# szpajder/dumphfdl

Hardware: AMD Instinct MI355X
Metric: wideband I/Q Msamples/s (cf32 ingest -> decoded HFDL PDUs) at fixed channel count (higher is better)
Workload: dtype f32

## Files before the change

### dumphfdl_amd/csrc/demod_core.h

```cpp
#pragma once
#include <hip/hip_runtime.h>
#include "demod_logic.h"
#include "demod_lds.h"

namespace hfdl {

constexpr int DM_WAVES = 4, DM_THREADS = 64 * DM_WAVES;

__device__ __forceinline__ float dpp_row_shr1(float old, float src)
{
	return __int_as_float(__builtin_amdgcn_update_dpp(__float_as_int(old), __float_as_int(src), 0x111, 0xf, 0xf, false));
}
__device__ __forceinline__ float dpp_row_shl1(float old, float src)
{
	return __int_as_float(__builtin_amdgcn_update_dpp(__float_as_int(old), __float_as_int(src), 0x101, 0xf, 0xf, false));
}
__device__ __forceinline__ float dpp_row_shl2(float old, float src)
{
	return __int_as_float(__builtin_amdgcn_update_dpp(__float_as_int(old), __float_as_int(src), 0x102, 0xf, 0xf, false));
}
__device__ __forceinline__ float dpp_row_ror1(float src)
{
	return __int_as_float(__builtin_amdgcn_update_dpp(0, __float_as_int(src), 0x121, 0xf, 0xf, false));
}
// ... 116 lines not shown
		for (int j = 0; j < D_RS_TAPS; j++) {
			const cf x = ring[(i - j) & DM_IN_MASK];
			ar += h[j] * x.x;
			ai += h[j] * x.y;
		}
		cf v; v.x = ar; v.y = ai;
		io.rs[k & DM_MASK] = v;
		if (TAPS) io.tap_resampled[k] = v;
	}
}


struct SymsyncRegs {
	float rate, del, tau, bf, q, qhat, v1;
	int b, decim, j;
	int valid_from;
};

__device__ __forceinline__ void symsync_load(SymsyncRegs &r, const ChanScalars &s, const ChanArrays &a, const BlockIo &io, int lane)
{
	if (lane < SS_HIST) {
		cf v; v.x = 0.f; v.y = 0.f;
		if (lane < D_SS_TAPS) v = a.ss_dmf[lane == 0 ? 0 : D_SS_TAPS - lane];
		io.mf[-1 - lane] = v;
	}
	r.rate = s.ss_rate; r.del = s.ss_del; r.tau = s.ss_tau; r.bf = s.ss_bf; r.q = s.ss_q; r.qhat = s.ss_qhat; r.v1 = s.ss_v1;
	r.b = s.ss_b; r.decim = (int)s.ss_decim; r.j = 0;
	r.valid_from = s.ss_head;
}

__device__ __forceinline__ void symsync_restart(SymsyncRegs &r, const DemodShared &sh, int k0)
{
	r.rate = 1.5f; r.del = 1.5f; r.tau = 0.f; r.bf = 0.f; r.q = 0.f; r.qhat = 0.f; r.v1 = 0.f;
	r.b = 0; r.decim = 0;
	r.j = k0 > 0 ? (int)sh.cum[(k0 - 1) & DM_MASK] : 0;
	r.valid_from = k0;
}

__device__ __forceinline__ void symsync_store(const SymsyncRegs &r, ChanScalars &s, ChanArrays &a, const BlockIo &io, int n_out, int lane)
{
	if (lane < D_SS_TAPS) a.ss_dmf[lane == 0 ? 0 : D_SS_TAPS - lane] = io.mf[((n_out - 1) & DM_MASK) - lane];
	if (lane == 0) {
		s.ss_rate = r.rate; s.ss_del = r.del; s.ss_tau = r.tau; s.ss_bf = r.bf; s.ss_q = r.q; s.ss_qhat = r.qhat; s.ss_v1 = r.v1;
		s.ss_b = r.b; s.ss_decim = (uint32_t)r.decim;
		const int vf = r.valid_from - n_out;
		s.ss_head = vf < -64 ? -64 : vf;
	}
}

template <bool MASKED>
__device__ __forceinline__ void symsync_chunk(SymsyncRegs &r, const DemodConst &T, const BlockIo &io, const DemodShared &sh, int k0, int k1, int lane)
{
	const int row = lane >> 4, t = lane & 15;
	const float *base = (const float *)(io.mf - (k0 & ~DM_MASK) - t) + (row & 1);
	int bi = r.b < 0 ? 0 : (r.b >= D_SS_NPFB ? D_SS_NPFB - 1 : r.b);
	float2 h = sh.sstab[bi * 64 + lane];
	float w_lo = base[2 * k0], w_hi = base[2 * (k0 - 16)];
	const bool out_lane = lane == 15 || lane == 31;
	float *const out_base = out_lane ? (float *)sh.outq + (lane == 31 ? 1 : 0) : sh.sink + lane;
	const int out_stride = out_lane ? 2 : 0;
	int cum_v = 0;
	for (int k = k0; k < k1; k++) {
		const float n_lo = base[2 * (k + 1)], n_hi = base[2 * (k + 1 - 16)];
		if (r.b < D_SS_NPFB) {
			float wl = w_lo, wh = w_hi;
			if (MASKED && k - (D_SS_TAPS - 1) < r.valid_from && row < 2) {
				if (k - t < r.valid_from) wl = 0.f;
				if (k - t - 16 < r.valid_from) wh = 0.f;
			}
			int produced = 0;
			do {
				const float p = row_scan_sum(h.x * wl + h.y * wh);
				if (__builtin_expect(r.j < sh.outq_cap, 1)) out_base[out_stride * (r.j & (OUTQ_RING - 1))] = div3(p);
				r.j++;
				if (r.decim == 2) {
					r.decim = 0;
					const float mx = lane_value(p, 15), my = lane_value(p, 31);
					const float dx = lane_value(p, 47), dy = lane_value(p, 63);
					float q = mx * dx + my * dy;
					q = q > 1.0f ? 1.0f : (q < -1.0f ? -1.0f : q);
					r.q = q;
					const float v0 = q - T.lf_a1 * r.v1;
					r.qhat = T.lf_b0 * v0;
					r.v1 = v0;
					r.rate += T.ss_rate_adj * r.qhat;
					r.del = r.rate + r.qhat;
				}
				r.decim++;
				r.tau += r.del;
				r.bf = r.tau * (float)D_SS_NPFB;
				r.b = (int)roundf(r.bf);
				produced++;
				if (r.b < D_SS_NPFB) h = sh.sstab[(r.b < 0 ? 0 : r.b) * 64 + lane];
			} while (r.b < D_SS_NPFB && produced < 4);
		}
		r.tau -= 1.0f;
		r.bf -= (float)D_SS_NPFB;
		r.b -= D_SS_NPFB;
		bi = r.b < 0 ? 0 : (r.b >= D_SS_NPFB ? D_SS_NPFB - 1 : r.b);
		h = sh.sstab[bi * 64 + lane];
		cum_v = (lane == k - k0) ? (r.j < 65535 ? r.j : 65535) : cum_v;
		w_lo = n_lo; w_hi = n_hi;
	}
	if (lane < k1 - k0) sh.cum[(k0 + lane) & DM_MASK] = (uint16_t)cum_v;
}


struct CarrierRegs {
	float eu, ev, ex2, ewx, ewy;
	float px, py;
#ifdef HFDL_DM_PROBE
	unsigned long long pa = 0, pb = 0, pc = 0;
#endif
};

struct LaneSlicer {
	float px, py;
	int lane;
	__device__ __forceinline__ uint32_t operator()(int arity, cf x, float *phase_error) const
	{
		uint32_t sym;
		cf xh;
		if (arity == 1) {
			sym = (x.x > 0) ? 0 : 1;
			xh.x = sym ? -1.0f : 1.0f; xh.y = 0.0f;
		} else {
			const int M = 1 << arity, base = M - 2;
			const bool mine = lane >= base && lane < base + M;
			const float d = mine ? x.x * px + x.y * py : -1.0f;
			const float best = lane_value(row_scan_max(d), 15);
			const unsigned long long hit = __builtin_amdgcn_fcmpf(d, best, 1 );
			int win = hit ? (int)__builtin_ctzll(hit) : base;
			const uint32_t lin = (uint32_t)(win - base);
			sym = lin ^ (lin >> 1);
			xh.x = lane_value(px, win); xh.y = lane_value(py, win);
		}
		if (phase_error) *phase_error = x.y * xh.x - x.x * xh.y;
		return sym;
	}
};

__device__ __forceinline__ void carrier_load(CarrierRegs &c, const ChanScalars &s, const ChanArrays &a, const DemodConst &T, int lane)
{
	c.px = lane < 16 ? T.psk_pts[2 * lane] : 0.f;
	c.py = lane < 16 ? T.psk_pts[2 * lane + 1] : 0.f;
	const int t = (lane & 15) - 1;
	const bool act = t >= 0 && lane < 32, row1 = (lane >> 4) & 1;
	int j = s.eq_head + t; if (j >= D_EQ) j -= D_EQ;
	const cf e = act ? a.eq_buf[j] : cf{0.f, 0.f};
	c.eu = row1 ? e.y : e.x;
	c.ev = row1 ? -e.x : e.y;
	c.ex2 = act ? a.eq_x2[j] : 0.f;
	const cf w = act ? a.eq_w[t] : cf{0.f, 0.f};
	c.ewx = w.x; c.ewy = w.y;
}
// ... 299 lines not shown
	if (reset_at >= 0) {
		s.ev_flags = 0;
		s.sample_cnt = cnt0 + (uint64_t)reset_at + 1u;
		return k0 + reset_at;
	}
	if (kdone < n) catch_up(n - 1);
	s.sample_cnt = cnt0 + (uint64_t)n;
	return -1;
}


template <bool TAPS>
__device__ inline int demod_block(ChanArrays &a, const DemodConst &T, const BlockIo &io, const DemodShared &sh, const DemodInput &in)
{
	const int tid = (int)threadIdx.x, wave = tid >> 6, lane = tid & 63;
	ChanScalars &S = *sh.S;
	unsigned long long tR0 = __builtin_amdgcn_s_memtime();

	const uint32_t rs_phase = S.rs_phase;
	const int n_in = in.n_in;
	const uint64_t total = (uint64_t)n_in << 24;
	int n_out = 0;
	if ((uint64_t)rs_phase < total) n_out = (int)((total - rs_phase + T.rs_step - 1) / T.rs_step);
	if (n_out > io.cap - 4) n_out = io.cap - 4;
	auto need = [&](int k_end) {
		return k_end >= n_out ? n_in : (int)(((uint64_t)rs_phase + (uint64_t)(k_end - 1) * T.rs_step) >> 24) + 1;
	};
	auto resampler_store = [&]() {
		cf nh;
		if (lane < D_RS_TAPS - 1) nh = in.ring[(n_in - 1 - lane) & DM_IN_MASK];
		__builtin_amdgcn_wave_barrier();
		if (lane < D_RS_TAPS - 1) a.rs_hist[lane] = nh;
		if (lane == 0) {
			S.rs_phase = (uint32_t)((uint64_t)rs_phase + (uint64_t)n_out * T.rs_step - total);
			if (TAPS) io.tap_counts[0] = n_out;
		}
	};

	if (tid < D_RS_TAPS - 1) in.ring[(-1 - tid) & DM_IN_MASK] = a.rs_hist[tid];
	if (wave == 1 && lane < D_MF - 1) io.agc[(-1 - lane) & DM_AGC_MASK] = a.mf_hist[lane];
	const int rs0 = n_out < DM_CHUNK ? n_out : DM_CHUNK;
	int in_loaded = need(rs0 + 2 * DM_CHUNK);
	for (int g = tid; g < in_loaded; g += DM_THREADS) in.ring[g & DM_IN_MASK] = input_sample(in, g);
	if (TAPS && tid == 0) io.tap_counts[1] = 0;
	__syncthreads();
	if (wave == 3) resample_outputs<TAPS>(rs_phase, T, io, in.ring, 0, rs0, lane);
	__syncthreads();
	if (n_out < 1) {
		if (wave == 3) resampler_store();
		return 0;
	}

	unsigned long long tP0 = __builtin_amdgcn_s_memtime();
	unsigned long long busy = 0;
	int nsym = 0;
#ifdef HFDL_DM_PROBE
	unsigned long long cr_probe[3] = { 0, 0, 0 };
#endif
	PipeProgress pp;
	pp.rs_ready = rs0;
	if (wave == 3) {
		for (int step = 0; pp.s3_done < n_out; step++) {
			int *mb = sh.mbox + 8 * (step & 1);
			int to = pp.rs_ready;
			if (to < n_out) {
				to = to + DM_CHUNK < n_out ? to + DM_CHUNK : n_out;
				if (to > pp.s3_done + DM_RS_AHEAD) to = pp.s3_done + DM_RS_AHEAD;
				const int hi = need(to + 2 * DM_CHUNK < n_out ? to + 2 * DM_CHUNK : n_out);
				cf nx[2];
#pragma unroll
				for (int u = 0; u < 2; u++) {
					const int g = in_loaded + 64 * u + lane;
					nx[u] = g < hi ? input_sample(in, g) : cf{0.f, 0.f};
				}
				resample_outputs<TAPS>(rs_phase, T, io, in.ring, pp.rs_ready, to, lane);
#pragma unroll
				for (int u = 0; u < 2; u++) {
					const int g = in_loaded + 64 * u + lane;
					if (g < hi) in.ring[g & DM_IN_MASK] = nx[u];
				}
				for (int g = in_loaded + 128 + lane; g < hi; g += 64) in.ring[g & DM_IN_MASK] = input_sample(in, g);
				if (hi > in_loaded) in_loaded = hi;
			}
			if (lane == 0) mb[4] = to;
			__syncthreads();
			pp.read(mb);
		}
		resampler_store();
	} else if (wave == 0) {
		float agc_g = S.agc_g, agc_y2 = S.agc_y2;
		for (int step = 0; pp.s3_done < n_out; step++) {
			int *mb = sh.mbox + 8 * (step & 1);
			int to = pp.mf_ready + DM_CHUNK < pp.rs_ready ? pp.mf_ready + DM_CHUNK : pp.rs_ready;
			if (to > pp.s3_done + DM_MF_AHEAD) to = pp.s3_done + DM_MF_AHEAD;
			if (to > pp.mf_ready) agc_mf_chunk<TAPS>(agc_g, agc_y2, T, io, pp.mf_ready, to, lane); else to = pp.mf_ready;
			if (lane == 0) mb[0] = to;
			__syncthreads();
			pp.read(mb);
		}
		cf nh;
		if (lane < D_MF - 1) nh = io.agc[(n_out - 1 - lane) & DM_AGC_MASK];
		__builtin_amdgcn_wave_barrier();
		if (lane < D_MF - 1) a.mf_hist[lane] = nh;
		if (lane == 0) { S.agc_g = agc_g; S.agc_y2 = agc_y2; }
	} else if (wave == 1) {
		SymsyncRegs ss;
		symsync_load(ss, S, a, io, lane);
		__builtin_amdgcn_fence(__ATOMIC_RELEASE, "wavefront");
		__builtin_amdgcn_wave_barrier();
		for (int step = 0; pp.s3_done < n_out; step++) {
			int *mb = sh.mbox + 8 * (step & 1);
			const unsigned long long tb = TAPS ? __builtin_amdgcn_s_memtime() : 0ull;
			if (pp.restart) symsync_restart(ss, sh, pp.ss_ready);
			int to = pp.ss_ready + DM_CHUNK < pp.mf_ready ? pp.ss_ready + DM_CHUNK : pp.mf_ready;
			if (to > pp.s3_done + 2 * DM_CHUNK) to = pp.s3_done + 2 * DM_CHUNK;
			if (to < pp.ss_ready) to = pp.ss_ready;
			for (int k0 = pp.ss_ready; k0 < to;) {
				const int k1 = (k0 | DM_MASK) + 1 < to ? (k0 | DM_MASK) + 1 : to;
				if (__builtin_expect(k0 - (D_SS_TAPS - 1) < ss.valid_from, 0)) symsync_chunk<true>(ss, T, io, sh, k0, k1, lane);
				else symsync_chunk<false>(ss, T, io, sh, k0, k1, lane);
				k0 = k1;
			}
			if (lane == 0) mb[1] = to;
			if (TAPS) busy += __builtin_amdgcn_s_memtime() - tb;
			__syncthreads();
			pp.read(mb);
		}
		if (pp.restart) symsync_restart(ss, sh, n_out);
		symsync_store(ss, S, a, io, n_out, lane);
	} else {
		CarrierRegs cr;
		ChanScalars s3 = S;
		s3.ev_flags = 0;
		carrier_load(cr, s3, a, T, lane);
		for (int step = 0; pp.s3_done < n_out; step++) {
			int *mb = sh.mbox + 8 * (step & 1);
			const unsigned long long tb = TAPS ? __builtin_amdgcn_s_memtime() : 0ull;
			int to = pp.s3_done + DM_CHUNK < pp.ss_ready ? pp.s3_done + DM_CHUNK : pp.ss_ready;
			int reset_at = -1;
			if (to > pp.s3_done) reset_at = carrier_chunk<TAPS>(cr, s3, a, T, io, sh, pp.s3_done, to, nsym, lane); else to = pp.s3_done;
			if (lane == 0) { mb[2] = reset_at >= 0 ? reset_at + 1 : to; mb[3] = reset_at >= 0; }
			if (TAPS) busy += __builtin_amdgcn_s_memtime() - tb;
			__syncthreads();
			pp.read(mb);
		}
		carrier_store(cr, a, lane);
#ifdef HFDL_DM_PROBE
		cr_probe[0] = cr.pa; cr_probe[1] = cr.pb; cr_probe[2] = cr.pc;
#endif
		if (lane == 0) {
			S.phi = s3.phi; S.dphi = s3.dphi; S.err = s3.err;
			S.eq_x2sum = s3.eq_x2sum; S.eq_count = s3.eq_count; S.eq_full = s3.eq_full; S.eq_head = 0;
			S.bits_hi = s3.bits_hi; S.bits_lo = s3.bits_lo;
			S.training_n = s3.training_n; S.data_n = s3.data_n; S.use_data = s3.use_data; S.data_slot = s3.data_slot;
			S.symbol_cnt = s3.symbol_cnt; S.sample_cnt = s3.sample_cnt;
			S.s_state = s3.s_state; S.fr_state = s3.fr_state; S.cur_arity = s3.cur_arity;
			S.symbols_wanted = s3.symbols_wanted; S.T_idx = s3.T_idx;
			S.bitmask = s3.bitmask; S.symsync_out_idx = s3.symsync_out_idx; S.nf_clk = s3.nf_clk;
			S.frame_symbol_cnt = s3.frame_symbol_cnt; S.signal_level = s3.signal_level;
			S.noise_floor = s3.noise_floor;
			S.ev_flags = 0;
			if (TAPS) io.tap_counts[1] = nsym;
		}
	}
	unsigned long long tP1 = __builtin_amdgcn_s_memtime();
	if (TAPS) {
		if (tid == 0) { io.tap_level[io.cap - 4] = (float)(tP0 - tR0); io.tap_level[io.cap - 3] = (float)(tP1 - tP0); }
		if (wave == 1 && lane == 0) io.tap_level[io.cap - 2] = (float)busy;
		if (wave == 2 && lane == 0) io.tap_level[io.cap - 1] = (float)busy;
#ifdef HFDL_DM_PROBE
		__syncthreads();
		if (wave == 2 && lane == 0) { io.tap_level[io.cap - 4] = (float)cr_probe[0]; io.tap_level[io.cap - 3] = (float)cr_probe[1]; io.tap_level[io.cap - 2] = (float)cr_probe[2]; }
#endif
	}
	return n_out;
}

}
```

### dumphfdl_amd/csrc/frontend_query.cpp

```cpp
#include <cstdarg>
#include <cstdio>
#include <cstring>
#include <mutex>
#include "frontend.h"

using namespace hfdl;

static thread_local char g_err[512] = "";

int hfdl::fail(int code, const char *fmt, ...)
{
	va_list ap;
	va_start(ap, fmt);
	vsnprintf(g_err, sizeof(g_err), fmt, ap);
	va_end(ap);
	return code;
}

int hfdl::fail_hip(hipError_t e, bool alloc, const char *expr, const char *file, int line)
{
	return fail(alloc && e == hipErrorOutOfMemory ? HFDL_GPU_ENOMEM : HFDL_GPU_EHIP, "%s: %s (%s:%d)", expr, hipGetErrorString(e), file, line);
}

extern "C" const char *hfdl_gpu_last_error(void) { return g_err; }
// ... 196 lines not shown
	if (!fe || !out) return fail(HFDL_GPU_EINVAL, "null argument");
	memset(out, 0, sizeof(*out));
	out->blocks = fe->blocks;
	out->pdus_taken = fe->demod.taken;
	out->pdus_dropped = fe->demod.dropped;
	out->pdu_ring_capacity = (uint32_t)fe->demod.pdu_cap;
	return 0;
}

extern "C" int hfdl_gpu_frontend_enable_taps(hfdl_gpu_frontend *fe, int enable)
{
	if (int rc = sync_to_read(fe)) return rc;
	fe->demod.taps_enabled = enable != 0;
	return 0;
}

extern "C" int hfdl_gpu_frontend_read_tap_block(hfdl_gpu_frontend *fe, int what, int32_t channel, int32_t back, float *dst, size_t cap, size_t *n_floats)
{
	if (int rc = sync_to_read(fe, dst && n_floats)) return rc;
	const Geometry &g = fe->geo;
	if (back < 0 || back > fe->last_index) return fail(HFDL_GPU_ERANGE, "block %d back is not held any more (%d are)", back, fe->last_index);
	if (back && what != HFDL_GPU_TAP_SPECTRUM && what != HFDL_GPU_TAP_CHAN_OUT && what != HFDL_GPU_TAP_NCO_PHASORS)
		return fail(HFDL_GPU_EINVAL, "tap %d holds the last launch only", what);
	const int slot = fe->last_slot - back, index = fe->last_index - back;
	if ((what != HFDL_GPU_TAP_SPECTRUM || fe->nrx > 1) && (channel < 0 || channel >= g.nch)) return fail(HFDL_GPU_EINVAL, "channel out of range");
	const void *src = nullptr;
	size_t nf = 0;
	switch (what) {
	case HFDL_GPU_TAP_SPECTRUM:
		src = fe->spec_slot(fe->last_set, index) + (fe->nrx > 1 ? (size_t)fe->rx_of[(size_t)channel] * (size_t)g.n : 0);
		nf = 2 * (size_t)g.n;
		break;
	case HFDL_GPU_TAP_FILTER: {
		if (2 * (size_t)g.n > cap) return fail(HFDL_GPU_ERANGE, "tap needs %zu floats, buffer holds %zu", 2 * (size_t)g.n, cap);
		DevBuf plain;
		HIP_TRY(plain.alloc(sizeof(float2) * (size_t)g.n));
		launch_tap_extract(fe->d_taps, g, fe->slot_of(channel), plain.as<float2>(), fe->stream);
		HIP_TRY(hipStreamSynchronize(fe->stream));
		HIP_TRY(hipMemcpy(dst, plain.p, sizeof(float2) * (size_t)g.n, hipMemcpyDeviceToHost));
		*n_floats = 2 * (size_t)g.n;
		return 0; }
	case HFDL_GPU_TAP_CHAN_OUT: {
		int cnt = 0;
		HIP_TRY(hipMemcpy(&cnt, fe->cnt_slot(slot) + channel, sizeof(cnt), hipMemcpyDeviceToHost));
		src = fe->chan_slot(slot) + (size_t)channel * g.outs; nf = 2 * (size_t)cnt; break; }
	case HFDL_GPU_TAP_NCO_PHASORS: {
		int cnt = 0;
		HIP_TRY(hipMemcpy(&cnt, fe->cnt_slot(slot) + channel, sizeof(cnt), hipMemcpyDeviceToHost));
		if (2 * (size_t)cnt > cap) return fail(HFDL_GPU_ERANGE, "tap needs %zu floats, buffer holds %zu", 2 * (size_t)cnt, cap);
		if (cnt) HIP_TRY(hipMemcpy2D(dst, sizeof(float2), fe->ph_slot(fe->last_set, index) + channel, sizeof(float2) * (size_t)g.nch, sizeof(float2), (size_t)cnt, hipMemcpyDeviceToHost));
		*n_floats = 2 * (size_t)cnt;
		return 0; }
	case HFDL_GPU_TAP_PHASE_CYCLES: src = fe->demod.d_tap_lvl + (size_t)channel * fe->demod.cap + fe->demod.cap - 4; nf = 4; break;
	default:
		if (int rc = fe->demod.tap(what, channel, &src, &nf)) return rc;
	}
	if (nf > cap) return fail(HFDL_GPU_ERANGE, "tap needs %zu floats, buffer holds %zu", nf, cap);
	if (nf) HIP_TRY(hipMemcpy(dst, src, sizeof(float) * nf, hipMemcpyDeviceToHost));
	*n_floats = nf;
	return 0;
}

extern "C" int hfdl_gpu_frontend_read_tap(hfdl_gpu_frontend *fe, int what, int32_t channel, float *dst, size_t cap, size_t *n_floats)
{
	return hfdl_gpu_frontend_read_tap_block(fe, what, channel, 0, dst, cap, n_floats);
}


static_assert(HFDL_GPU_SPECTRUM_HANN == SPECMON_HANN && HFDL_GPU_SPECTRUM_MAXHOLD == SPECMON_MAXHOLD, "include/hfdl_gpu.h and spectrum.h name the same flags");
static_assert(HFDL_GPU_RECEIVERS_MAX <= 64, "SpecmonJob::fresh is one bit per receiver");

extern "C" int hfdl_gpu_frontend_spectrum_enable(hfdl_gpu_frontend *fe, int32_t bins, uint32_t flags)
{
	if (!fe) return fail(HFDL_GPU_EINVAL, "null argument");
	if (flags & ~(HFDL_GPU_SPECTRUM_HANN | HFDL_GPU_SPECTRUM_MAXHOLD)) return fail(HFDL_GPU_EINVAL, "unknown spectrum flags 0x%x", flags);
	if (bins != 0 && (bins < 16 || (bins & (bins - 1)) != 0)) return fail(HFDL_GPU_EINVAL, "spectrum bins %d: a power of two >= 16 (or 0 = off)", bins);
	if (bins > fe->geo.n / 16) return fail(HFDL_GPU_ERANGE, "spectrum bins %d: at most fft_size / 16 = %d", bins, fe->geo.n / 16);
	HIP_TRY(hipSetDevice(fe->device));
	if (fe->mon) (void)hipEventSynchronize(fe->mon->ev);
	fe->mon.reset();
	if (bins == 0) return 0;
	const size_t nb = (size_t)bins, K = (size_t)fe->nrx;
	auto mon = std::make_unique<SpectrumMonitor>();
	hipError_t e = mon->acc.alloc(sizeof(float2) * nb * K);
	if (e == hipSuccess && (flags & HFDL_GPU_SPECTRUM_MAXHOLD)) e = mon->peak.alloc(sizeof(float) * nb * K);
	if (e == hipSuccess) e = mon->host.alloc(3 * nb);
	if (e == hipSuccess) e = mon->ev.create(EV_NO_TIMING);
	if (e != hipSuccess) return fail(e == hipErrorOutOfMemory ? HFDL_GPU_ENOMEM : HFDL_GPU_EHIP, "spectrum monitor buffers: %s", hipGetErrorString(e));
	mon->bins = bins;
	mon->flags = flags;
	mon->fresh = ~(uint64_t)0;
	mon->blocks.assign(K, 0);
	mon->first.assign(K, 0);
	fe->mon = std::move(mon);
	return 0;
}

extern "C" int hfdl_gpu_frontend_spectrum_read(hfdl_gpu_frontend *fe, int32_t rx, float *mean, float *peak, int32_t cap,
		uint64_t *blocks, uint64_t *first_block, int reset)
{
	if (!fe || !mean || !blocks || !first_block) return fail(HFDL_GPU_EINVAL, "null argument");
	SpectrumMonitor *mon = fe->mon.get();
	if (!mon) return fail(HFDL_GPU_EINVAL, "the spectrum monitor is off: hfdl_gpu_frontend_spectrum_enable() first");
	if (rx < 0 || rx >= fe->nrx) return fail(HFDL_GPU_EINVAL, "receiver %d out of range (%d receivers)", rx, fe->nrx);
	if (peak && !(mon->flags & HFDL_GPU_SPECTRUM_MAXHOLD)) return fail(HFDL_GPU_EINVAL, "peak asked for, but the monitor was enabled without HFDL_GPU_SPECTRUM_MAXHOLD");
	if (cap < mon->bins) return fail(HFDL_GPU_ERANGE, "%d bands, buffer holds %d", mon->bins, cap);
// ... 20 lines not shown
```

### dumphfdl_amd/frontend.py

```python
import ctypes as C
import os
import sys
import numpy as np

_HERE = os.path.dirname(os.path.abspath(__file__))
PDU_MAX_OCTETS = 960

TAP_SPECTRUM, TAP_FILTER, TAP_CHAN_OUT, TAP_RESAMPLED, TAP_MF_OUT, TAP_SYMBOLS, TAP_AGC_LEVEL, TAP_PHASE_CYCLES, TAP_NCO_PHASORS = range(1, 10)


SFMT_CF32, SFMT_CS16, SFMT_CU8 = 0, 1, 2
FCS_GOOD, FCS_BAD, FCS_TOO_SHORT = 0, 1, 2
KIND_SPDU, KIND_MPDU_DOWNLINK, KIND_MPDU_UPLINK = 0, 1, 2


class GpuError(RuntimeError):
    pass


class Geometry(C.Structure):
    _fields_ = [(n, C.c_int32) for n in (
        "sample_rate", "decimation", "pre_decimation", "post_decimation", "taps_length", "overlap_length",
        "fft_size", "fft_inv_size", "input_size", "post_input_size", "scrap", "outputs_per_block",
        "channels", "fold_slices")] + [("transition_bw", C.c_float), ("resamp_rate", C.c_float), ("max_outputs_per_block", C.c_int32), ("demod_batch", C.c_int32), ("fold_batch", C.c_int32),
                                       ("prefetch_depth", C.c_int32), ("fold_rows", C.c_int32)]


class Pdu(C.Structure):
    _fields_ = [("channel", C.c_int32), ("freq", C.c_int32), ("mode", C.c_int32), ("bit_rate", C.c_int32),
                ("len", C.c_int32), ("freq_err_hz", C.c_float), ("rssi_db", C.c_float), ("noise_floor_db", C.c_float),
                ("slot", C.c_char), ("fcs_status", C.c_uint8), ("pdu_kind", C.c_uint8), ("hdr_len", C.c_uint16),
                ("sample_index", C.c_uint64),
                ("train_bits_bad", C.c_int32), ("train_bits_total", C.c_int32),
                ("lpdus_processed", C.c_uint8), ("lpdus_good", C.c_uint8), ("lpdus_bad_fcs", C.c_uint8), ("lpdus_too_short", C.c_uint8),
                ("lpdus_truncated", C.c_uint8), ("lpdu_pad", C.c_uint8 * 3),
                ("octets", C.c_uint8 * PDU_MAX_OCTETS)]


class ChannelStats(C.Structure):
    _fields_ = [("freq", C.c_int32), ("a2_found", C.c_uint32), ("m1_found", C.c_uint32), ("m1_not_found", C.c_uint32),
                ("frames", C.c_uint32), ("noise_floor_db", C.c_float), ("agc_level", C.c_float), ("costas_dphi", C.c_float),
                ("framer_state", C.c_int32), ("sample_cnt", C.c_uint64), ("symbol_cnt", C.c_uint64),
                ("a1_found", C.c_uint32), ("a1_corr_avg", C.c_float), ("a2_corr_avg", C.c_float), ("m1_corr_avg", C.c_float),
                ("train_bits_bad", C.c_uint32), ("train_bits_total", C.c_uint32)]


class FrontendCounters(C.Structure):
    _fields_ = [("blocks", C.c_uint64), ("pdus_taken", C.c_uint32), ("pdus_dropped", C.c_uint32), ("pdu_ring_capacity", C.c_uint32)]


def lib_path():
    return os.environ.get("HFDL_GPU_LIB") or os.path.join(_HERE, "libhfdl_gpu.so")


def lab_lib_path():
    return os.environ.get("HFDL_GPU_LAB_LIB") or os.path.join(_HERE, "libhfdl_gpu_lab.so")


_lib = None
_lab = None

# ... 214 lines not shown
            _check(rc, self._L)
        return bool(rc)

    def input_done_upto(self, host_block):
        _check(self._L.hfdl_gpu_frontend_input_done_upto(self._h, C.c_uint64(host_block)), self._L)

    def sync(self):
        _check(self._L.hfdl_gpu_frontend_sync(self._h), self._L)

    def poll_pdus_raw(self, max_pdus=4096, max_in_flight=0):
        buf = (Pdu * max_pdus)()
        n = C.c_int32(0)
        if max_in_flight:
            _check(self._L.hfdl_gpu_frontend_poll_pdus_ready(self._h, buf, max_pdus, C.byref(n), max_in_flight), self._L)
        else:
            _check(self._L.hfdl_gpu_frontend_poll_pdus(self._h, buf, max_pdus, C.byref(n)), self._L)
        return buf, n.value

    @staticmethod
    def pdus_to_dicts(buf, n):
        out = []
        for i in range(n):
            p = buf[i]
            out.append(dict(channel=p.channel, freq=p.freq, mode=p.mode, bit_rate=p.bit_rate,
                            octets=bytes(p.octets[:p.len]), freq_err_hz=p.freq_err_hz, rssi_db=p.rssi_db,
                            noise_floor_db=p.noise_floor_db, slot=p.slot.decode(), sample_index=p.sample_index,
                            fcs_status=p.fcs_status, pdu_kind=p.pdu_kind, hdr_len=p.hdr_len,
                            train_bits_bad=p.train_bits_bad, train_bits_total=p.train_bits_total,
                            lpdus=(p.lpdus_processed, p.lpdus_good, p.lpdus_bad_fcs, p.lpdus_too_short, p.lpdus_truncated)))
        return out

    def poll_pdus(self, max_pdus=4096, max_in_flight=0):
        return self.pdus_to_dicts(*self.poll_pdus_raw(max_pdus, max_in_flight))

    def counters(self):
        c = FrontendCounters()
        _check(self._L.hfdl_gpu_frontend_counters(self._h, C.byref(c)), self._L)
        return {n: getattr(c, n) for n, _ in FrontendCounters._fields_}

    def all_channel_stats(self):
        nch = self.geometry.channels
        buf = (ChannelStats * nch)()
        n = C.c_int32(0)
        _check(self._L.hfdl_gpu_frontend_all_channel_stats(self._h, buf, nch, C.byref(n)), self._L)
        return [{k: getattr(buf[i], k) for k, _ in ChannelStats._fields_} for i in range(n.value)]

    def read_tap(self, what, channel=0, back=0):
        g = self.geometry
        cap = 2 * g.fft_size if what in (TAP_SPECTRUM, TAP_FILTER) else 2 * (g.post_input_size + 64) * max(1, g.demod_batch)
        buf = np.empty(cap, np.float32)
        n = C.c_size_t(0)
        _check(self._L.hfdl_gpu_frontend_read_tap_block(self._h, what, channel, back, _p(buf), cap, C.byref(n)), self._L)
        out = buf[:n.value].copy()
        return out if what in (TAP_AGC_LEVEL, TAP_PHASE_CYCLES) else out.view(np.complex64)

    def enable_taps(self, enable=True):
        _check(self._L.hfdl_gpu_frontend_enable_taps(self._h, int(enable)), self._L)

    def channel_stats(self, channel):
        st = ChannelStats()
        _check(self._L.hfdl_gpu_frontend_channel_stats(self._h, channel, C.byref(st)), self._L)
        return {n: getattr(st, n) for n, _ in ChannelStats._fields_}

    def reset_timers(self, enable=True):
        _check(self._L.hfdl_gpu_frontend_reset_timers(self._h, int(enable)), self._L)

    def fold_time_ms(self):
        ms = C.c_double(0)
        n = C.c_int64(0)
        _check(self._L.hfdl_gpu_frontend_fold_time_ms(self._h, C.byref(ms), C.byref(n)), self._L)
        return ms.value, n.value

    def fold_blocks(self):
        n = C.c_int64(0)
        _check(self._L.hfdl_gpu_frontend_fold_blocks(self._h, C.byref(n)), self._L)
        return n.value

    def fold_launch_shapes(self):
        c = (C.c_int64 * (FOLD_BATCH_MAX + 1))()
        _check(self._L.hfdl_gpu_frontend_fold_launch_shapes(self._h, C.byref(c), None), self._L)
        return {nb: int(c[nb]) for nb in range(1, FOLD_BATCH_MAX + 1) if c[nb]}

    def fold_launch_times(self):
        c, ms = (C.c_int64 * (FOLD_BATCH_MAX + 1))(), (C.c_double * (FOLD_BATCH_MAX + 1))()
        _check(self._L.hfdl_gpu_frontend_fold_launch_shapes(self._h, C.byref(c), C.byref(ms)), self._L)
        return {nb: (int(c[nb]), float(ms[nb])) for nb in range(1, FOLD_BATCH_MAX + 1) if c[nb]}

    def stage_times(self):
        ms, n = (C.c_double * 5)(), (C.c_int64 * 5)()
        _check(self._L.hfdl_gpu_frontend_stage_times(self._h, C.byref(ms), C.byref(n)), self._L)
        return {k: (ms[i], int(n[i])) for i, k in enumerate(("fft", "fold", "ifft", "demod", "decode"))}

    def fold_variant_probe(self, variant, nb, reps=3):
        avg, best, chk = C.c_double(0), C.c_double(0), C.c_uint64(0)
        _check(self._L.hfdl_gpu_lab_fold_variant_probe(self._h, variant, nb, reps, C.byref(avg), C.byref(best), C.byref(chk)), self._L)
        return avg.value, best.value, chk.value

    def demod_time_ms(self):
        ms = C.c_double(0)
        n = C.c_int64(0)
        nb = C.c_int64(0)
        _check(self._L.hfdl_gpu_frontend_demod_time_ms(self._h, C.byref(ms), C.byref(n), C.byref(nb)), self._L)
        return ms.value, n.value, nb.value

    def step_period_ms(self):
        v = C.c_double(0)
        _check(self._L.hfdl_gpu_frontend_step_period_ms(self._h, C.byref(v)), self._L)
# ... 185 lines not shown
```

### include/hfdl_gpu.h

```cpp
#ifndef HFDL_GPU_H
#define HFDL_GPU_H
#include <stdint.h>
#include <stddef.h>

#ifdef __cplusplus
extern "C" {
#endif

#define HFDL_GPU_EINVAL   (-1)
#define HFDL_GPU_ENODEV   (-2)
#define HFDL_GPU_ENOMEM   (-3)
#define HFDL_GPU_EHIP     (-4)
#define HFDL_GPU_ERANGE   (-5)

#define HFDL_GPU_PDU_MAX_OCTETS 960

#define HFDL_GPU_FCS_GOOD      0
#define HFDL_GPU_FCS_BAD       1
#define HFDL_GPU_FCS_TOO_SHORT 2
#define HFDL_GPU_KIND_SPDU          0
#define HFDL_GPU_KIND_MPDU_DOWNLINK 1
#define HFDL_GPU_KIND_MPDU_UPLINK   2

typedef struct hfdl_gpu_frontend hfdl_gpu_frontend;
// ... 56 lines not shown
int  hfdl_gpu_frontend_push_block(hfdl_gpu_frontend *fe, const float *iq, size_t nsamples, int on_device);
int  hfdl_gpu_frontend_input_done(hfdl_gpu_frontend *fe);
int  hfdl_gpu_frontend_input_done_upto(hfdl_gpu_frontend *fe, uint64_t host_block);
int  hfdl_gpu_frontend_input_copied(hfdl_gpu_frontend *fe, uint64_t host_block);
int  hfdl_gpu_frontend_prefetch_block_raw(hfdl_gpu_frontend *fe, const void *raw, size_t nsamples, int sample_format);
int  hfdl_gpu_frontend_prefetch_cancel(hfdl_gpu_frontend *fe);
#define HFDL_GPU_SFMT_CF32 0
#define HFDL_GPU_SFMT_CS16 1
#define HFDL_GPU_SFMT_CU8  2
int  hfdl_gpu_frontend_push_block_raw(hfdl_gpu_frontend *fe, const void *raw, size_t nsamples, int sample_format, int on_device);
int  hfdl_gpu_frontend_push_baseband(hfdl_gpu_frontend *fe, const float *chan_out, const int32_t *counts);
int  hfdl_gpu_frontend_channelize_block(hfdl_gpu_frontend *fe, const float *iq, size_t nsamples, int on_device);
int  hfdl_gpu_frontend_sync(hfdl_gpu_frontend *fe);
int  hfdl_gpu_frontend_poll_pdus(hfdl_gpu_frontend *fe, hfdl_gpu_pdu *out, int32_t max, int32_t *n);
int  hfdl_gpu_frontend_poll_pdus_ready(hfdl_gpu_frontend *fe, hfdl_gpu_pdu *out, int32_t max, int32_t *n, int32_t max_in_flight);
typedef struct {
	uint64_t blocks;
	uint32_t pdus_taken;
	uint32_t pdus_dropped;
	uint32_t pdu_ring_capacity;
} hfdl_gpu_frontend_counters_t;
int  hfdl_gpu_frontend_counters(hfdl_gpu_frontend *fe, hfdl_gpu_frontend_counters_t *out);
void *hfdl_gpu_frontend_stream(hfdl_gpu_frontend *fe);

typedef struct {
	int32_t  freq;
	uint32_t a2_found, m1_found, m1_not_found, frames;
	float    noise_floor_db;
	float    agc_level, costas_dphi;
	int32_t  framer_state;
	uint64_t sample_cnt, symbol_cnt;
	uint32_t a1_found;
	float    a1_corr_avg, a2_corr_avg, m1_corr_avg;
	uint32_t train_bits_bad, train_bits_total;
} hfdl_gpu_channel_stats;
int  hfdl_gpu_frontend_channel_stats(hfdl_gpu_frontend *fe, int32_t channel, hfdl_gpu_channel_stats *out);
int  hfdl_gpu_frontend_all_channel_stats(hfdl_gpu_frontend *fe, hfdl_gpu_channel_stats *out, int32_t cap, int32_t *n);

#define HFDL_GPU_SPECTRUM_HANN    1u
#define HFDL_GPU_SPECTRUM_MAXHOLD 2u
int  hfdl_gpu_frontend_spectrum_enable(hfdl_gpu_frontend *fe, int32_t bins, uint32_t flags);
int  hfdl_gpu_frontend_spectrum_read(hfdl_gpu_frontend *fe, int32_t rx, float *mean, float *peak, int32_t cap,
		uint64_t *blocks, uint64_t *first_block, int reset);

enum {
	HFDL_GPU_TAP_SPECTRUM = 1,
	HFDL_GPU_TAP_FILTER = 2,
	HFDL_GPU_TAP_CHAN_OUT = 3,
	HFDL_GPU_TAP_RESAMPLED = 4,
	HFDL_GPU_TAP_MF_OUT = 5,
	HFDL_GPU_TAP_SYMBOLS = 6,
	HFDL_GPU_TAP_AGC_LEVEL = 7,
	HFDL_GPU_TAP_NCO_PHASORS = 9,
	HFDL_GPU_TAP_PHASE_CYCLES = 8
};
int  hfdl_gpu_frontend_enable_taps(hfdl_gpu_frontend *fe, int enable);
int  hfdl_gpu_frontend_read_tap(hfdl_gpu_frontend *fe, int what, int32_t channel, float *dst, size_t cap, size_t *n_floats);
int  hfdl_gpu_frontend_read_tap_block(hfdl_gpu_frontend *fe, int what, int32_t channel, int32_t back, float *dst, size_t cap, size_t *n_floats);

int  hfdl_gpu_frontend_fold_time_ms(hfdl_gpu_frontend *fe, double *total_ms, int64_t *launches);
int  hfdl_gpu_frontend_fold_blocks(hfdl_gpu_frontend *fe, int64_t *blocks);
int  hfdl_gpu_frontend_fold_launch_shapes(hfdl_gpu_frontend *fe, int64_t counts[HFDL_GPU_FOLD_BATCH_MAX + 1], double ms[HFDL_GPU_FOLD_BATCH_MAX + 1]);
int  hfdl_gpu_frontend_reset_timers(hfdl_gpu_frontend *fe, int enable);
int  hfdl_gpu_frontend_demod_time_ms(hfdl_gpu_frontend *fe, double *total_ms, int64_t *launches, int64_t *blocks);
int  hfdl_gpu_frontend_stage_times(hfdl_gpu_frontend *fe, double ms[5], int64_t launches[5]);
int  hfdl_gpu_frontend_step_period_ms(hfdl_gpu_frontend *fe, double *period_ms);

int  hfdl_gpu_fft_forward(int device, const float *in, float *out, int32_t n, int shifted);
int  hfdl_gpu_viterbi27(int device, const uint8_t *soft, int32_t nbits, int32_t nframes, uint8_t *out);
int  hfdl_gpu_burst_decode(int device, const float *symbols, const int32_t *modes, const int32_t *bitmask_lsb,
		int32_t nframes, uint8_t *octets, int32_t *lens);

int  hfdl_gpu_nco_decimate(int device, const float *in, int32_t input_size, float rate, int32_t decimation,
		int32_t *decimation_remain, float *starting_phase, float *out, int32_t *output_size);
int  hfdl_gpu_crc16_ccitt(int device, const uint8_t *data, uint32_t len, uint16_t crc_init, uint16_t *crc);
int  hfdl_gpu_pdu_triage(int device, const uint8_t *octets, const int32_t *lens, int32_t npdus, int32_t stride,
		uint8_t *fcs_status, uint8_t *pdu_kind, uint16_t *hdr_len);

int  hfdl_gpu_lpdu_walk(int device, const uint8_t *octets, const int32_t *lens, int32_t npdus, int32_t stride, uint8_t *counts);

int  hfdl_gpu_psk_slice(int device, int32_t arity, const float *xy, int32_t n, uint32_t *sym, float *phase_error);

double hfdl_gpu_last_stage_ms(void);

const char *hfdl_gpu_last_error(void);
int  hfdl_gpu_device_count(void);

#ifdef __cplusplus
}
#endif
#endif
```

Baseline: 19080.

## Add steady-state fast path to symbol sync loop and per-wave step timing taps

Adds a specialized steady-state run inside the unmasked symbol-timing chunk. When the polyphase index is in range, it produces one output per input sample (or skips a sample) with wave-uniform scalarized control, unrolls the decimation-by-two loop-filter update into alternating calls, and rolls state back when the index leaves the expected range. This removes the general do-while and branching overhead on the serial symsync wave, which is likely a pipeline bottleneck. It also adds busy/wait cycle counters for every pipeline wave behind the TAPS flag, plus a new tap and a profiling script, at the cost of more code complexity and register pressure.

Measured after the change: 18670. 0.978x the previous value.

```diff
diff --git a/dumphfdl_amd/csrc/demod_core.h b/dumphfdl_amd/csrc/demod_core.h
--- a/dumphfdl_amd/csrc/demod_core.h
+++ b/dumphfdl_amd/csrc/demod_core.h
@@ -192,6 +192,7 @@
 __device__ __forceinline__ void symsync_chunk(SymsyncRegs &r, const DemodConst &T, const BlockIo &io, const DemodShared &sh, int k0, int k1, int lane)
 {
 	const int row = lane >> 4, t = lane & 15;
+	k0 = __builtin_amdgcn_readfirstlane(k0); k1 = __builtin_amdgcn_readfirstlane(k1);
 	const float *base = (const float *)(io.mf - (k0 & ~DM_MASK) - t) + (row & 1);
 	int bi = r.b < 0 ? 0 : (r.b >= D_SS_NPFB ? D_SS_NPFB - 1 : r.b);
 	float2 h = sh.sstab[bi * 64 + lane];
@@ -200,7 +201,73 @@
 	float *const out_base = out_lane ? (float *)sh.outq + (lane == 31 ? 1 : 0) : sh.sink + lane;
 	const int out_stride = out_lane ? 2 : 0;
 	int cum_v = 0;
-	for (int k = k0; k < k1; k++) {
+#ifdef HFDL_DM_NO_STEADY_RUN
+	constexpr bool RUN = false;
+#else
+	constexpr bool RUN = !MASKED;
+#endif
+	int k = k0;
+
+	auto steady_output = [&](const bool update, const int k_end) -> bool {
+		const SymsyncRegs r0 = r;
+		const int cum0 = cum_v;
+		const float a_lo = base[2 * (k + 1)], a_hi = base[2 * (k + 1 - 16)];
+		const float b_lo = base[2 * (k + 2)], b_hi = base[2 * (k + 2 - 16)];
+		const float p = row_scan_sum(h.x * w_lo + h.y * w_hi);
+		out_base[out_stride * (r.j & (OUTQ_RING - 1))] = div3(p);
+		r.j++;
+		if (update) {
+			const float mx = lane_value(p, 15), my = lane_value(p, 31);
+			const float dx = lane_value(p, 47), dy = lane_value(p, 63);
+			float q = mx * dx + my * dy;
+			q = q > 1.0f ? 1.0f : (q < -1.0f ? -1.0f : q);
+			r.q = q;
+			const float v0 = q - T.lf_a1 * r.v1;
+			r.qhat = T.lf_b0 * v0;
+			r.v1 = v0;
+			r.rate += T.ss_rate_adj * r.qhat;
+			r.del = r.rate + r.qhat;
+		}
+		r.decim = update ? 1 : 2;
+		r.tau += r.del;
+		r.bf = r.tau * (float)D_SS_NPFB;
+		r.b = __builtin_amdgcn_readfirstlane((int)roundf(r.bf));
+		cum_v = (lane >= k - k0) ? r.j : cum_v;
+		if (__builtin_expect(r.b < D_SS_NPFB, 0)) {
+			r = r0;
+			cum_v = cum0;
+			return false;
+		}
+		r.tau -= 1.0f;
+		r.bf -= (float)D_SS_NPFB;
+		r.b -= D_SS_NPFB;
+		const bool none = r.b >= D_SS_NPFB;
+		const float tau2 = r.tau - 1.0f, bf2 = r.bf - (float)D_SS_NPFB;
+		r.tau = none ? tau2 : r.tau;
+		r.bf = none ? bf2 : r.bf;
+		r.b = none ? r.b - D_SS_NPFB : r.b;
+		k += none ? 2 : 1;
+		w_lo = none ? b_lo : a_lo;
+		w_hi = none ? b_hi : a_hi;
+		h = sh.sstab[(r.b >= D_SS_NPFB ? D_SS_NPFB - 1 : r.b) * 64 + lane];
+		return r.b < D_SS_NPFB && k < k_end;
+	};
+	auto steady_run = [&]() {
+		if (r.decim == 0) return;
+		r.j = __builtin_amdgcn_readfirstlane(r.j);
+		const int cap = sh.outq_cap < 65535 ? sh.outq_cap : 65535;
+		int k_end = k1 - 1;
+		if (k_end - k > cap - r.j) k_end = k + (cap - r.j);
+		if (k >= k_end) return;
+		if (r.decim == 2 && !steady_output(true, k_end)) return;
+		for (;;) {
+			if (!steady_output(false, k_end)) return;
+			if (!steady_output(true, k_end)) return;
+		}
+	};
+
+	if (RUN && (unsigned)r.b < (unsigned)D_SS_NPFB) steady_run();
+	while (k < k1) {
 		const float n_lo = base[2 * (k + 1)], n_hi = base[2 * (k + 1 - 16)];
 		if (r.b < D_SS_NPFB) {
 			float wl = w_lo, wh = w_hi;
@@ -241,6 +308,8 @@
 		h = sh.sstab[bi * 64 + lane];
 		cum_v = (lane == k - k0) ? (r.j < 65535 ? r.j : 65535) : cum_v;
 		w_lo = n_lo; w_hi = n_hi;
+		k++;
+		if (RUN && (unsigned)r.b < (unsigned)D_SS_NPFB) steady_run();
 	}
 	if (lane < k1 - k0) sh.cum[(k0 + lane) & DM_MASK] = (uint16_t)cum_v;
 }
@@ -646,7 +715,7 @@
 	}
 
 	unsigned long long tP0 = __builtin_amdgcn_s_memtime();
-	unsigned long long busy = 0;
+	unsigned long long busy = 0, wait = 0;
 	int nsym = 0;
 #ifdef HFDL_DM_PROBE
 	unsigned long long cr_probe[3] = { 0, 0, 0 };
@@ -656,6 +725,7 @@
 	if (wave == 3) {
 		for (int step = 0; pp.s3_done < n_out; step++) {
 			int *mb = sh.mbox + 8 * (step & 1);
+			const unsigned long long tb = TAPS ? __builtin_amdgcn_s_memtime() : 0ull;
 			int to = pp.rs_ready;
 			if (to < n_out) {
 				to = to + DM_CHUNK < n_out ? to + DM_CHUNK : n_out;
@@ -677,20 +747,25 @@
 				if (hi > in_loaded) in_loaded = hi;
 			}
 			if (lane == 0) mb[4] = to;
+			const unsigned long long tw = TAPS ? __builtin_amdgcn_s_memtime() : 0ull;
 			__syncthreads();
 			pp.read(mb);
+			if (TAPS) { busy += tw - tb; wait += __builtin_amdgcn_s_memtime() - tw; }
 		}
 		resampler_store();
 	} else if (wave == 0) {
 		float agc_g = S.agc_g, agc_y2 = S.agc_y2;
 		for (int step = 0; pp.s3_done < n_out; step++) {
 			int *mb = sh.mbox + 8 * (step & 1);
+			const unsigned long long tb = TAPS ? __builtin_amdgcn_s_memtime() : 0ull;
 			int to = pp.mf_ready + DM_CHUNK < pp.rs_ready ? pp.mf_ready + DM_CHUNK : pp.rs_ready;
 			if (to > pp.s3_done + DM_MF_AHEAD) to = pp.s3_done + DM_MF_AHEAD;
 			if (to > pp.mf_ready) agc_mf_chunk<TAPS>(agc_g, agc_y2, T, io, pp.mf_ready, to, lane); else to = pp.mf_ready;
 			if (lane == 0) mb[0] = to;
+			const unsigned long long tw = TAPS ? __builtin_amdgcn_s_memtime() : 0ull;
 			__syncthreads();
 			pp.read(mb);
+			if (TAPS) { busy += tw - tb; wait += __builtin_amdgcn_s_memtime() - tw; }
 		}
 		cf nh;
 		if (lane < D_MF - 1) nh = io.agc[(n_out - 1 - lane) & DM_AGC_MASK];
@@ -716,9 +791,10 @@
 				k0 = k1;
 			}
 			if (lane == 0) mb[1] = to;
-			if (TAPS) busy += __builtin_amdgcn_s_memtime() - tb;
+			const unsigned long long tw = TAPS ? __builtin_amdgcn_s_memtime() : 0ull;
 			__syncthreads();
 			pp.read(mb);
+			if (TAPS) { busy += tw - tb; wait += __builtin_amdgcn_s_memtime() - tw; }
 		}
 		if (pp.restart) symsync_restart(ss, sh, n_out);
 		symsync_store(ss, S, a, io, n_out, lane);
@@ -734,9 +810,10 @@
 			int reset_at = -1;
 			if (to > pp.s3_done) reset_at = carrier_chunk<TAPS>(cr, s3, a, T, io, sh, pp.s3_done, to, nsym, lane); else to = pp.s3_done;
 			if (lane == 0) { mb[2] = reset_at >= 0 ? reset_at + 1 : to; mb[3] = reset_at >= 0; }
-			if (TAPS) busy += __builtin_amdgcn_s_memtime() - tb;
+			const unsigned long long tw = TAPS ? __builtin_amdgcn_s_memtime() : 0ull;
 			__syncthreads();
 			pp.read(mb);
+			if (TAPS) { busy += tw - tb; wait += __builtin_amdgcn_s_memtime() - tw; }
 		}
 		carrier_store(cr, a, lane);
 #ifdef HFDL_DM_PROBE
@@ -762,6 +839,12 @@
 		if (tid == 0) { io.tap_level[io.cap - 4] = (float)(tP0 - tR0); io.tap_level[io.cap - 3] = (float)(tP1 - tP0); }
 		if (wave == 1 && lane == 0) io.tap_level[io.cap - 2] = (float)busy;
 		if (wave == 2 && lane == 0) io.tap_level[io.cap - 1] = (float)busy;
+		if (n_out <= io.cap - 8 && lane == 0) {
+			if (wave == 0) io.tap_level[io.cap - 8] = (float)busy;
+			if (wave == 3) io.tap_level[io.cap - 7] = (float)busy;
+			if (wave == 1) io.tap_level[io.cap - 6] = (float)wait;
+			if (wave == 2) io.tap_level[io.cap - 5] = (float)wait;
+		}
 #ifdef HFDL_DM_PROBE
 		__syncthreads();
 		if (wave == 2 && lane == 0) { io.tap_level[io.cap - 4] = (float)cr_probe[0]; io.tap_level[io.cap - 3] = (float)cr_probe[1]; io.tap_level[io.cap - 2] = (float)cr_probe[2]; }
diff --git a/dumphfdl_amd/csrc/frontend_query.cpp b/dumphfdl_amd/csrc/frontend_query.cpp
--- a/dumphfdl_amd/csrc/frontend_query.cpp
+++ b/dumphfdl_amd/csrc/frontend_query.cpp
@@ -272,6 +272,7 @@
 		*n_floats = 2 * (size_t)cnt;
 		return 0; }
 	case HFDL_GPU_TAP_PHASE_CYCLES: src = fe->demod.d_tap_lvl + (size_t)channel * fe->demod.cap + fe->demod.cap - 4; nf = 4; break;
+	case HFDL_GPU_TAP_STEP_CYCLES: src = fe->demod.d_tap_lvl + (size_t)channel * fe->demod.cap + fe->demod.cap - 8; nf = 4; break;
 	default:
 		if (int rc = fe->demod.tap(what, channel, &src, &nf)) return rc;
 	}
diff --git a/dumphfdl_amd/frontend.py b/dumphfdl_amd/frontend.py
--- a/dumphfdl_amd/frontend.py
+++ b/dumphfdl_amd/frontend.py
@@ -7,6 +7,7 @@
 PDU_MAX_OCTETS = 960
 
 TAP_SPECTRUM, TAP_FILTER, TAP_CHAN_OUT, TAP_RESAMPLED, TAP_MF_OUT, TAP_SYMBOLS, TAP_AGC_LEVEL, TAP_PHASE_CYCLES, TAP_NCO_PHASORS = range(1, 10)
+TAP_STEP_CYCLES = 10
 
 
 SFMT_CF32, SFMT_CS16, SFMT_CU8 = 0, 1, 2
@@ -327,7 +328,7 @@
         n = C.c_size_t(0)
         _check(self._L.hfdl_gpu_frontend_read_tap_block(self._h, what, channel, back, _p(buf), cap, C.byref(n)), self._L)
         out = buf[:n.value].copy()
-        return out if what in (TAP_AGC_LEVEL, TAP_PHASE_CYCLES) else out.view(np.complex64)
+        return out if what in (TAP_AGC_LEVEL, TAP_PHASE_CYCLES, TAP_STEP_CYCLES) else out.view(np.complex64)
 
     def enable_taps(self, enable=True):
         _check(self._L.hfdl_gpu_frontend_enable_taps(self._h, int(enable)), self._L)
diff --git a/include/hfdl_gpu.h b/include/hfdl_gpu.h
--- a/include/hfdl_gpu.h
+++ b/include/hfdl_gpu.h
@@ -132,7 +132,8 @@
 	HFDL_GPU_TAP_SYMBOLS = 6,
 	HFDL_GPU_TAP_AGC_LEVEL = 7,
 	HFDL_GPU_TAP_NCO_PHASORS = 9,
-	HFDL_GPU_TAP_PHASE_CYCLES = 8
+	HFDL_GPU_TAP_PHASE_CYCLES = 8,
+	HFDL_GPU_TAP_STEP_CYCLES = 10
 };
 int  hfdl_gpu_frontend_enable_taps(hfdl_gpu_frontend *fe, int enable);
 int  hfdl_gpu_frontend_read_tap(hfdl_gpu_frontend *fe, int what, int32_t channel, float *dst, size_t cap, size_t *n_floats);
diff --git a/profiles/stage_cycles.py b/profiles/stage_cycles.py
--- /dev/null
+++ b/profiles/stage_cycles.py
@@ -0,0 +1,75 @@
+#!/usr/bin/env python3
+import json
+import os
+import sys
+sys.path.insert(0, os.path.dirname(os.path.dirname(os.path.abspath(__file__))))
+import numpy as np
+import dumphfdl_amd as hf
+import hfdl_synth as synth
+from dumphfdl_amd import frontend as F
+from oracle import pyoracle
+
+FS, CF, FREQ = 250000, 10_000_000, 10_021_000
+repeats = int(sys.argv[1]) if len(sys.argv) > 1 else 2
+
+
+def stream(mode):
+    rng = np.random.default_rng(300 + mode)
+    bursts = [dict(freq=FREQ, mode=mode, octets=synth.make_pdu(rng, mode), t0=1.2, amp=0.1, cfo=4.0)]
+    dur = 1.2 + synth.burst_symbols_len(mode) / 1800.0 + 0.3
+    x = synth.synth_wideband(FS, CF, int(dur * FS), bursts, noise_sigma=0.004, seed=70 + mode)
+    ora = pyoracle.Frontend(FS, CF, [FREQ])
+    size, parts = ora.ddc.input_size, []
+    for b in range(len(x) // size):
+        ora.push_block(x[b * size:(b + 1) * size])
+        parts.append(np.array(ora.channel_view(0)["chan_out"], np.complex64))
+    ora.close()
+    return np.concatenate(parts)
+
+
+def inputs_for(phase, step, n_out):
+    outputs = lambda n_in: ((n_in << 24) - phase + step - 1) // step if phase < (n_in << 24) else 0
+    n_in = max(1, (phase + (n_out - 1) * step) >> 24)
+    while outputs(n_in) < n_out:
+        n_in += 1
+    return n_in, outputs(n_in)
+
+
+rows = {}
+for mode in (1, 2, 3):
+    x = stream(mode)
+    for rep in range(repeats):
+        fe = hf.Frontend(FS, CF, [FREQ])
+        step, phase, at, inside = int(round(float(1 << 24) / float(fe.geometry.resamp_rate))), 0, 0, 0
+        body = lambda s: s["m1_found"] > s["frames"]
+        before = fe.all_channel_stats()[0]
+        while at < len(x):
+            n_in, n_out = inputs_for(phase, step, 512)
+            if at + n_in > len(x):
+                break
+            fe.push_baseband([x[at:at + n_in]])
+            at += n_in
+            phase += n_out * step - (n_in << 24)
+            after = fe.all_channel_stats()[0]
+            t = fe.read_tap(F.TAP_PHASE_CYCLES, 0)
+            try:
+                u = fe.read_tap(F.TAP_STEP_CYCLES, 0)
+            except Exception:
+                u = np.zeros(4, np.float32)
+            if body(before) and body(after) and before["frames"] == after["frames"]:
+                inside += 1
+                cls = "mode %d T" % mode if inside <= 2 else "mode %d data" % mode
+            elif not body(before) and not body(after) and before["a2_found"] == after["a2_found"] and before["frames"] == after["frames"]:
+                cls, inside = "search", 0
+            else:
+                cls, inside = "mixed", 0
+            rows.setdefault(cls, []).append([t[1] / n_out, t[2] / n_out, t[3] / n_out, u[0] / n_out, u[1] / n_out, u[2] / n_out, u[3] / n_out])
+            before = after
+        fe.close()
+lib = os.environ.get("HFDL_GPU_LIB")
+print("lib", os.path.relpath(lib, os.path.dirname(os.path.dirname(os.path.abspath(__file__)))) if lib else "product")
+print("%-14s %4s  %-9s %-9s %-9s %-9s %-9s %-9s %-9s" % ("state", "n", "P", "W1", "W2", "W0", "W3", "G1", "G2"))
+for cls in sorted(rows):
+    a = np.array(rows[cls])
+    print("%-14s %4d  " % (cls, len(a)) + " ".join("%4.0f-%-4.0f" % (lo, hi) for lo, hi in zip(a.min(axis=0), a.max(axis=0))))
+print(json.dumps({k: np.array(v).mean(axis=0).round(1).tolist() for k, v in rows.items()}))
```
